# liuhuang31/Megatts2_HierSpeechpp

Hardware: AMD Instinct MI355X
Metric: 16kHz audio samples/sec (whole node) + RTF, HierSpeech++ vocoder batch=32 (higher is better)
Workload: dtype f32; 1 GPU; vocoder-only infer(): 32 utterances x 4 s per GPU (BASELINE.json configs[1]), synthetic weights; batch_per_gpu=32, frames=200, global_batch=32, parallelism=dp1 (contiguous utterance shards of the global batch, one RCCL weight broadcast), launch_mode=hipGraph replay of the captured step

## Files before the change

### megatts2_hierspeechpp_amd/csrc/hsp_dftseg.hip

```cpp
#include "hsp_device.h"
#include <algorithm>
#include <cmath>

namespace {
typedef float ds_f32x16 __attribute__((ext_vector_type(16)));
typedef float ds_f32x4 __attribute__((ext_vector_type(4)));
constexpr int DS_N = 128, DS_H = 64;
constexpr int DS_MEM = 256;
#define DS_ACC_ROW(r, half) (((r) & 3) + 8 * ((r) >> 2) + 4 * (half))

struct DsCol {
  int ch, p, s;
  bool ok;
};
__device__ __forceinline__ DsCol ds_col(int col, int ncols, int d, int S) {
  DsCol c;
  c.ok = col < ncols;
  const int cc = c.ok ? col : ncols - 1;
  const int per = d * S;
  c.ch = cc / per;
  const int rem = cc - c.ch * per;
  c.p = rem / S;
  c.s = rem - c.p * S;
  return c;
}

struct DsGeom {
  int cg, S, pitch, ngrp, nchunk, bufsz;
};
struct DsItem {
  int b, c0, ncg, s0, S;
};
__device__ __forceinline__ DsItem ds_item(int item, const hsp_dftseg_args& a, const DsGeom& G) {
  DsItem I;
  const int id = item / G.nchunk, sc = item - id * G.nchunk;
  I.b = id / G.ngrp;
  I.c0 = (id - I.b * G.ngrp) * G.cg;
  I.ncg = min(G.cg, a.C - I.c0);
  I.s0 = sc * G.S;
  I.S = min(G.S, a.nseg - I.s0);
  return I;
}
__device__ __forceinline__ void ds_barrier() { asm volatile("s_waitcnt lgkmcnt(0)\n\ts_barrier" ::: "memory"); }

__device__ __forceinline__ unsigned ds_lds_addr(const float* p) {
  return (unsigned)(size_t)(const __attribute__((address_space(3))) float*)p;
}
__device__ __forceinline__ void ds_rd(float& dst, unsigned addr) { asm volatile("ds_read_b32 %0, %1" : "=v"(dst) : "v"(addr)); }
template <int OFF>
__device__ __forceinline__ void ds_rd_at(float& dst, unsigned addr) {
  static_assert(OFF >= 0 && OFF < 65536, "ds_read immediate offsets are 16 bits");
// ... 53 lines not shown
  const float inv_ng = 1.0f / (float)s.ng;
#pragma unroll
  for (int u = 0; u < 16; ++u) {
    const int e = e0 + t + DS_MEM * u, ch = s.tot == s.ng ? 0 : ds_div(min(e, s.tot - 1), s.ng, inv_ng), gi = e - ch * s.ng;
    if (e < s.tot) *reinterpret_cast<ds_f32x4*>(buf + ch * G.pitch + s.sh - s.t0 + 4 * (s.g_lo + gi)) = v[u];
  }
}

constexpr int DA_SEG = 240, DA_RAW = 256, DA_A2 = 496, DA_SLICE = DA_RAW + DA_A2;
typedef float ds_f32x2 __attribute__((ext_vector_type(2)));
__device__ __forceinline__ void da_fence() { asm volatile("" ::: "memory"); }
struct DaItem {
  int pa, pb, pa4, nsg, nsegs;
};
template <bool RAG = false>
__device__ __forceinline__ DaItem da_item(const hsp_dftseg_args& a, const DsItem& I, const DsStage& s, int lb = 0) {
  const int L = RAG ? lb : a.L;
  DaItem A;
  A.pa = max(s.t0, 0);
  A.pb = min(s.t0 + s.len, L);
  A.pa4 = A.pa & ~3;
  A.nsg = (A.pb - A.pa4 + DA_SEG - 1) / DA_SEG;
  A.nsegs = I.ncg * A.nsg;
  if constexpr (RAG) {
    A.nsg = max(A.nsg, 1);
    A.nsegs = A.pb > A.pa ? I.ncg * A.nsg : 0;
  }
  return A;
}
template <bool RAG = false>
__device__ __forceinline__ ds_f32x4 da_load(const hsp_dftseg_args& a, const DsItem& I, const DaItem& A, int sI, int lane) {
  const int q = RAG ? max(min(sI, A.nsegs - 1), 0) : min(sI, A.nsegs - 1), ch = q / A.nsg, p0 = A.pa4 + DA_SEG * (q - ch * A.nsg);
  const float* xr = a.x + (int64_t)I.b * a.x_bs + (int64_t)(I.c0 + ch) * a.x_cs;
  return *reinterpret_cast<const ds_f32x4*>(xr + hsp_clampi(p0 - 8 + 4 * lane, 0, a.L - 4));
}
template <bool RAG = false>
__device__ __forceinline__ void da_segment(const hsp_dftseg_args& a, const DsGeom& G, const DsItem& I, const DsStage& s,
                                           const DaItem& A, int sI, int lane, ds_f32x4 rv, float* slice, float* buf,
                                           const float* flt, float add = 0.0f, int lb = 0, const float* last = nullptr,
                                           int64_t last_cs = 0) {
  const int ch = sI / A.nsg, p0 = A.pa4 + DA_SEG * (sI - ch * A.nsg);
  const int L = RAG ? lb : a.L;
  const int n_out = min(DA_SEG, L - p0);
  const int c = I.c0 + ch;
  const float kf = a.act_alpha_exp[c] * 0.318309886183790672f, kb = 0.5f * a.act_beta_inv[c];
  float* raw = slice;
  float* a2 = slice + DA_RAW;
  ds_f32x2 hu[6], hd[6];
#pragma unroll
  for (int i = 0; i < 6; ++i) {
    hu[i] = *reinterpret_cast<const ds_f32x2*>(flt + 2 * i);
    hd[i] = *reinterpret_cast<const ds_f32x2*>(flt + 12 + 2 * i);
  }
  {
    const int idx = p0 - 8 + 4 * lane;
    ds_f32x4 t = rv + add;
    t = idx < 0 ? ds_f32x4{t.x, t.x, t.x, t.x} : t;
    t = idx >= a.L ? ds_f32x4{t.w, t.w, t.w, t.w} : t;
    if constexpr (RAG) {
      const float rl = last[ch * last_cs] + add;
      t.x = idx >= L ? rl : t.x;
      t.y = idx + 1 >= L ? rl : t.y;
      t.z = idx + 2 >= L ? rl : t.z;
      t.w = idx + 3 >= L ? rl : t.w;
    }
    *reinterpret_cast<ds_f32x4*>(raw + 4 * lane) = t;
  }
  da_fence();
  const int npairs = (2 * n_out + 13) >> 2;
#pragma unroll
  for (int it = 0; it < 2; ++it) {
    const int pi = lane + 64 * it;
    if (pi < npairs) {
      const ds_f32x2* rp = reinterpret_cast<const ds_f32x2*>(raw + 2 * pi + 2);
      const ds_f32x2 r0 = rp[0], r1 = rp[1], r2 = rp[2], r3 = rp[3];
      const float xv[7] = {r0.y, r1.x, r1.y, r2.x, r2.y, r3.x, r3.y};
      ds_f32x2 u0 = {0.0f, 0.0f}, u1 = {0.0f, 0.0f};
#pragma unroll
      for (int i = 0; i < 6; ++i) {
        u0 = __builtin_elementwise_fma(ds_f32x2{xv[i], xv[i]}, hu[i], u0);
        u1 = __builtin_elementwise_fma(ds_f32x2{xv[i + 1], xv[i + 1]}, hu[i], u1);
      }
      *reinterpret_cast<ds_f32x4*>(a2 + 4 * pi) =
          ds_f32x4{hsp_snake_hw(u0.x, kf, kb), hsp_snake_hw(u0.y, kf, kb), hsp_snake_hw(u1.x, kf, kb), hsp_snake_hw(u1.y, kf, kb)};
    }
  }
  da_fence();
  if constexpr (RAG) {
    const int e = 2 * (L - p0) + 4;
    const bool tail = e < 2 * n_out + 9;
    if (p0 == 0 || tail) {
      if (p0 == 0 && lane < 5) a2[lane] = a2[5];
      if (tail && lane >= 8 && lane < 13) a2[e + lane - 7] = a2[e];
      da_fence();
    }
  } else if (p0 == 0 || p0 + n_out == a.L) {
    if (p0 == 0 && lane < 5) a2[lane] = a2[5];
    if (p0 + n_out == a.L && lane >= 8 && lane < 13) a2[2 * n_out + lane - 3] = a2[2 * n_out + 4];
    da_fence();
  }
  float* row = buf + ch * G.pitch + s.sh - s.t0;
#pragma unroll
  for (int it = 0; it < 2; ++it) {
    const int l2 = lane + 64 * it;
    if (2 * l2 < n_out) {
      const ds_f32x4* ap = reinterpret_cast<const ds_f32x4*>(a2 + 4 * l2);
      const ds_f32x4 q0 = ap[0], q1 = ap[1], q2 = ap[2];
      const ds_f32x2 q3 = *reinterpret_cast<const ds_f32x2*>(a2 + 4 * l2 + 12);
      const ds_f32x2 aw[7] = {{q0.x, q0.y}, {q0.z, q0.w}, {q1.x, q1.y}, {q1.z, q1.w}, {q2.x, q2.y}, {q2.z, q2.w}, q3};
      ds_f32x2 s0 = {0.0f, 0.0f}, s1 = {0.0f, 0.0f};
#pragma unroll
      for (int k = 0; k < 6; ++k) {
        s0 = __builtin_elementwise_fma(aw[k], hd[k], s0);
        s1 = __builtin_elementwise_fma(aw[k + 1], hd[k], s1);
      }
      const int p = p0 + 2 * l2;
      if (p >= A.pa && p < A.pb) row[p] = s0.x + s0.y;
      if (p + 1 >= A.pa && p + 1 < A.pb) row[p + 1] = s1.x + s1.y;
    }
  }
  da_fence();
}

template <bool ACT, bool RAG = false>
__global__ __launch_bounds__(DS_MEM) __attribute__((amdgpu_waves_per_eu(2, 2))) void dftseg_fwd_kernel(const hsp_dftseg_args a, const DsGeom G) {
  extern __shared__ __attribute__((aligned(16))) float lds[];
  const int tid = threadIdx.x, lane = tid & 63, wave = __builtin_amdgcn_readfirstlane(tid >> 6);
  const int l32 = lane & 31, half = lane >> 5;
  const int hop = DS_N - (a.k - 1), d = a.dil, pitch = G.pitch;
  const int nitems = a.B * G.ngrp * G.nchunk;
  const int nmine = (nitems - (int)blockIdx.x + (int)gridDim.x - 1) / (int)gridDim.x;
  const int wh = wave & 1, pairw = wave >> 1;
  float fa[32];
  {
    const float* frow = a.dft + (32 * wh + l32) * DS_H + half;
#pragma unroll
    for (int ks = 0; ks < 32; ++ks) fa[ks] = frow[2 * ks];
  }
  float* const twl = lds + G.bufsz;
  if (tid < 64) twl[tid] = a.dft[DS_H * DS_H + tid];
  float ov[32];
  bool pok = false;
  unsigned lb1 = 0, lb2 = 0, lbz = 0;
  const unsigned rowb = 4u * (unsigned)a.xf_bs, imb = 4u * (unsigned)(a.C * a.Np);
  const int lanek = 16 * wh + 4 * half;
  auto put = [&](int i) __attribute__((always_inline)) {
    const int r = i >> 2, w = i & 3;
    const unsigned cr = (unsigned)((r & 3) + 8 * (r >> 2)) * rowb;
    unsigned off = w < 2 ? lb1 + cr : lb2 - cr;
    if (r == 0 && w >= 2) off = lanek == 0 ? lbz : off;
    if (w & 1) off += imb;
    if (pok) *reinterpret_cast<float*>(reinterpret_cast<char*>(a.xf) + off) = ov[i];
  };
  const bool vec = ((a.L | (int)a.x_bs | (int)a.x_cs) & 3) == 0 && (reinterpret_cast<uintptr_t>(a.x) & 15) == 0;
  constexpr bool act = ACT;
  float* const flt = lds + G.bufsz + 64;
  float* const slice = flt + 32 + wave * DA_SLICE;
  if (act && tid < 24) {
    const int i = tid >> 1;
    flt[tid] = tid < 12 ? 2.0f * a.act_filt[10 - 2 * i + (tid & 1)] : a.act_filt[tid];
  }
  if (act) __syncthreads();
  DsItem I = ds_item(blockIdx.x, a, G);
  DsStage sg = ds_stage_of(a, I);
  auto row_len = [&](const DsItem& It) __attribute__((always_inline)) {
    return RAG ? (int)min(max(a.act_len[It.b], (int64_t)1), (int64_t)a.L) : a.L;
  };
  int lb = row_len(I);
  DaItem da = da_item<RAG>(a, I, sg, lb);
  ds_f32x4 pv[16];
  auto prefetch = [&]() __attribute__((always_inline)) {
    if (act) {
#pragma unroll
      for (int i = 0; i < 16; ++i) pv[i] = da_load<RAG>(a, I, da, wave + 4 * i, lane);
    } else if (vec) {
      ds_stage_load(a, I, sg, 0, tid, pv);
    }
  };
  prefetch();
  for (int it = 0; it < nmine; ++it) {
    if (it) ds_barrier();
    if (act) {
      const float* last = RAG ? a.x + (int64_t)I.b * a.x_bs + (int64_t)I.c0 * a.x_cs + (lb - 1) : nullptr;
#pragma unroll
      for (int i = 0; i < 16; ++i)
        if (wave + 4 * i < da.nsegs)
          da_segment<RAG>(a, G, I, sg, da, wave + 4 * i, lane, pv[i], slice, lds, flt, 0.0f, lb, last, a.x_cs);
      for (int sI = wave + 64; sI < da.nsegs; sI += 4)
        da_segment<RAG>(a, G, I, sg, da, sI, lane, da_load<RAG>(a, I, da, sI, lane), slice, lds, flt, 0.0f, lb, last, a.x_cs);
      for (int ch = 0; ch < I.ncg; ++ch) {
        float* row = lds + ch * pitch + sg.sh;
        for (int j = tid; j < min(-sg.t0, sg.len); j += DS_MEM) row[j] = 0.0f;
        for (int j = max((RAG ? lb : a.L) - sg.t0, 0) + tid; j < sg.len; j += DS_MEM) row[j] = 0.0f;
      }
    } else if (vec) {
      ds_stage_write(G, sg, 0, tid, lds, pv);
      for (int e0 = DS_MEM * 16; e0 < sg.tot; e0 += DS_MEM * 16) {
        ds_f32x4 v[16];
        ds_stage_load(a, I, sg, e0, tid, v);
        ds_stage_write(G, sg, e0, tid, lds, v);
      }
      for (int ch = 0; ch < I.ncg; ++ch) {
        float* row = lds + ch * pitch + sg.sh;
        for (int j = tid; j < min(-sg.t0, sg.len); j += DS_MEM) row[j] = 0.0f;
        for (int j = max(a.L - sg.t0, 0) + tid; j < sg.len; j += DS_MEM) row[j] = 0.0f;
      }
    } else {
      for (int ch = 0; ch < I.ncg; ++ch) {
        const float* xr = a.x + (int64_t)I.b * a.x_bs + (int64_t)(I.c0 + ch) * a.x_cs;
        float* row = lds + ch * pitch + sg.sh;
        for (int j0 = 0; j0 < sg.len; j0 += DS_MEM * 16) {
          float v[16];
#pragma unroll
          for (int u = 0; u < 16; ++u) v[u] = xr[min(max(sg.t0 + j0 + tid + DS_MEM * u, 0), a.L - 1)];
#pragma unroll
          for (int u = 0; u < 16; ++u) {
            const int j = j0 + tid + DS_MEM * u, ti = sg.t0 + j;
            if (j < sg.len) row[j] = (ti >= 0 && ti < a.L) ? v[u] : 0.0f;
          }
        }
      }
    }
    ds_barrier();
    const DsItem Ic = I;
    const int shc = sg.sh;
    if (it + 1 < nmine) {
      I = ds_item(blockIdx.x + (it + 1) * gridDim.x, a, G);
      sg = ds_stage_of(a, I);
      lb = row_len(I);
      da = da_item<RAG>(a, I, sg, lb);
      prefetch();
    }
    const int S = Ic.S, ncols = Ic.ncg * d * S;
    const float ipc = 1.0f / (float)(d * S), isc = 1.0f / (float)S;
    const float* buf = lds + shc;
    const int step = 4 * d;
    for (int cb = 32 * pairw; cb < ncols; cb += 64) {
      const DsCol q = ds_col_f(cb + l32, ncols, d, S, ipc, isc);
      const float* bp = buf + q.ch * pitch + q.p + d * (q.s * hop + 2 * half);
      ds_f32x16 ae, ao;
#pragma unroll
      for (int r = 0; r < 16; ++r) ae[r] = ao[r] = 0.0f;
      float rb[2][8];
      unsigned pe = ds_lds_addr(bp), po = pe + 4u * d;
      const unsigned st = 4u * step;
      auto issue = [&](float (&r)[8]) __attribute__((always_inline)) {
#pragma unroll
        for (int j = 0; j < 4; ++j) {
          ds_rd(r[2 * j], pe);
          ds_rd(r[2 * j + 1], po);
          pe += st;
          po += st;
        }
      };
      issue(rb[0]);
#pragma unroll
      for (int g = 0; g < 8; ++g) {
        ds_wait<0>(rb[g & 1]);
        if (g + 1 < 8) issue(rb[(g + 1) & 1]);
#pragma unroll
        for (int j = 0; j < 4; ++j) {
          ae = __builtin_amdgcn_mfma_f32_32x32x2f32(fa[4 * g + j], rb[g & 1][2 * j], ae, 0, 0, 0);
          ao = __builtin_amdgcn_mfma_f32_32x32x2f32(fa[4 * g + j], rb[g & 1][2 * j + 1], ao, 0, 0, 0);
          put(4 * g + j);
        }
      }
#pragma unroll
      for (int r = 0; r < 8; ++r) {
        const float er = ae[r], ei = ae[r + 8], orr = ao[r], oi = ao[r + 8];
        const float wc = twl[lanek + (r & 3) + 8 * (r >> 2)], ws = twl[32 + lanek + (r & 3) + 8 * (r >> 2)];
        const float tr = wc * orr + ws * oi, ti = wc * oi - ws * orr;
        const bool z = r == 0 && wh == 0 && half == 0;
        const bool z3 = z && a.prod3;
        ov[4 * r + 0] = z3 ? -er : er + tr;
        ov[4 * r + 1] = z ? (a.prod3 ? -tr : er - tr) : ei + ti;
        ov[4 * r + 2] = z ? ei : er - tr;
        ov[4 * r + 3] = z ? -oi : ti - ei;
      }
      {
        const unsigned colb = 4u * (unsigned)((Ic.c0 + q.ch) * a.Np + (Ic.b * d + q.p) * a.nseg + Ic.s0 + q.s);
        pok = q.ok;
        lb1 = colb + (unsigned)lanek * rowb;
        lb2 = colb + (unsigned)(64 - lanek) * rowb;
        lbz = colb + 32u * rowb;
      }
    }
  }
#pragma unroll
  for (int i = 0; i < 32; ++i) put(i);
}


template <int W, int U, bool RES, bool ACC>
__device__ __forceinline__ void ds_inv_epilogue_t(const hsp_dftseg_args& a, const DsGeom& G, const DsItem& I, const float* buf,
                                                  int w, int nw, int lane, int tb, int tl) {
  typedef float vec_t __attribute__((ext_vector_type(W)));
  const int nel = tl / W;
  const int R = (nel + 64 * U - 1) / (64 * U);
  const float ps = a.post_scale;
  int ch = 0, rr = w;
  while (rr >= R) rr -= R, ++ch;
  while (ch < I.ncg) {
    const int c = I.c0 + ch;
    const float bz = a.bias ? a.bias[c] : 0.0f;
// ... 176 lines not shown
    else ds_inv_epilogue<1, 4>(a, G, I, lds, wave, 4, lane, tb, tl);
    if (++it_c < nmine) {
      blk_c = 0;
      I = item_of(it_c);
      ncols = I.ncg * d * I.S;
    } else {
      done = true;
    }
  };
  float v1[16], v2[16];
  DsCol q1, q2;
  fetch_next(v1, q1);
  fetch_next(v2, q2);
  while (true) {
    step(v1, q1);
    if (done) break;
    step(v2, q2);
    if (done) break;
  }
}

struct DpGeom {
  int cg, ngrp, S1, pitchA, S2, pitchB, offB, offX, offT;
};

template <bool RAG = false>
__global__ __launch_bounds__(512) __attribute__((amdgpu_waves_per_eu(2, 2))) void dftseg_pair_kernel(
    const hsp_dftseg_args ai, const hsp_dftseg_args af, const DpGeom G) {
  extern __shared__ __attribute__((aligned(16))) float lds[];
  const int tid = threadIdx.x, lane = tid & 63, wave = __builtin_amdgcn_readfirstlane(tid >> 6);
  const int l32 = lane & 31, half = lane >> 5;
  const int hop1 = DS_N - (ai.k - 1), d1 = ai.dil, hop2 = DS_N - (af.k - 1), d2 = af.dil;
  float* const sA = lds;
  float* const sB = lds + G.offB;
  float* const twl = lds + G.offT;
  float* const flt = twl + 64;
  const int grp = wave >> 2, w4 = wave & 3, wh1 = w4 & 1, eo = w4 >> 1;
  const int pw = wave >> 1, wh3 = wave & 1;
  float* const bbuf = lds + G.offX + grp * (128 * 32);
  float* const slice = lds + G.offX + wave * DA_SLICE;
  float fa1[32], fa3[32], twc[4], tws[4];
  {
    const float* frow = ai.dft + (32 * wh1 + l32) * DS_H + half;
#pragma unroll
    for (int ks = 0; ks < 32; ++ks) fa1[ks] = frow[2 * ks];
    const float* grow = af.dft + (32 * wh3 + l32) * DS_H + half;
#pragma unroll
    for (int ks = 0; ks < 32; ++ks) fa3[ks] = grow[2 * ks];
// ... 64 lines not shown
#pragma unroll
      for (int ks = 0; ks < 32; ks += 2) {
        acc = __builtin_amdgcn_mfma_f32_32x32x2f32(fa1[ks], bp[ks * 64], acc, 0, 0, 0);
        acc2 = __builtin_amdgcn_mfma_f32_32x32x2f32(fa1[ks + 1], bp[ks * 64 + 64], acc2, 0, 0, 0);
      }
      if (q.ok) ds_inv_scatter(sA + q.ch * G.pitchA + q.p + d1 * (q.s * hop1 + i0), d1, i0, hop1, wh1, acc, acc2);
      ds_barrier();
    };
    for (int st = 0; st < nst; ++st) {
      if (odd) step1(v2, q2);
      else step1(v1, q1);
      odd = !odd;
    }
    {
      DsStage sg;
      sg.t0 = -af.pad;
      sg.len = d2 * ((G.S2 - 1) * hop2 + DS_N);
      sg.sh = 4 + (sg.t0 & 3);
      sg.g_lo = 0;
      sg.ng = 0;
      sg.tot = 0;
      const int lb = RAG ? (int)min(max(af.act_len[I.b], (int64_t)1), (int64_t)af.L) : af.L;
      const DaItem da = da_item<RAG>(af, I, sg, lb);
      for (int sI = wave; sI < da.nsegs; sI += 8) {
        const int ch = sI / da.nsg, p0 = da.pa4 + DA_SEG * (sI - ch * da.nsg);
        const ds_f32x4 rv = *reinterpret_cast<const ds_f32x4*>(sA + ch * G.pitchA + hsp_clampi(p0 - 8 + 4 * lane, 0, af.L - 4));
        da_segment<RAG>(af, Gf, I, sg, da, sI, lane, rv, slice, sB, flt, ai.bias ? ai.bias[I.c0 + ch] : 0.0f,
                        lb, sA + (lb - 1), G.pitchA);
      }
      for (int ch = 0; ch < I.ncg; ++ch) {
        float* row = sB + ch * G.pitchB + sg.sh;
        for (int j = tid; j < min(-sg.t0, sg.len); j += 512) row[j] = 0.0f;
        for (int j = max(lb - sg.t0, 0) + tid; j < sg.len; j += 512) row[j] = 0.0f;
      }
      ds_barrier();
      const int ncols2 = I.ncg * d2 * G.S2;
      const float* buf = sB + sg.sh;
      const int step = 4 * d2;
      const unsigned rowb = 4u * (unsigned)af.xf_bs, imb = 4u * (unsigned)(af.C * af.Np);
      const int lanek = 16 * wh3 + 4 * half;
      const float ip2 = 1.0f / (float)(d2 * G.S2), is2 = 1.0f / (float)G.S2;
      for (int cb = 32 * pw; cb < ncols2; cb += 128) {
        const DsCol q = ds_col_f(cb + l32, ncols2, d2, G.S2, ip2, is2);
        const float* bp = buf + q.ch * G.pitchB + q.p + d2 * (q.s * hop2 + 2 * half);
        ds_f32x16 ae, ao;
#pragma unroll
        for (int r = 0; r < 16; ++r) ae[r] = ao[r] = 0.0f;
#pragma unroll
        for (int ks = 0; ks < 32; ++ks) {
          ae = __builtin_amdgcn_mfma_f32_32x32x2f32(fa3[ks], bp[ks * step], ae, 0, 0, 0);
          ao = __builtin_amdgcn_mfma_f32_32x32x2f32(fa3[ks], bp[ks * step + d2], ao, 0, 0, 0);
        }
        if (q.ok) {
          const unsigned colb = 4u * (unsigned)((I.c0 + q.ch) * af.Np + (I.b * d2 + q.p) * af.nseg + q.s);
          char* const base = reinterpret_cast<char*>(af.xf);
#pragma unroll
          for (int r = 0; r < 8; ++r) {
            const int kr = (r & 3) + 8 * (r >> 2);
            const float er = ae[r], ei = ae[r + 8], orr = ao[r], oi = ao[r + 8];
            const float wc = twl[lanek + kr], ws = twl[32 + lanek + kr];
            const float tr = wc * orr + ws * oi, ti = wc * oi - ws * orr;
            const bool z = r == 0 && lanek == 0;
            const bool z3 = z && af.prod3;
            const unsigned o1 = colb + (unsigned)(lanek + kr) * rowb;
            const unsigned o2 = colb + (z ? 32u : (unsigned)(64 - lanek - kr)) * rowb;
            *reinterpret_cast<float*>(base + o1) = z3 ? -er : er + tr;
            *reinterpret_cast<float*>(base + o1 + imb) = z ? (af.prod3 ? -tr : er - tr) : ei + ti;
            *reinterpret_cast<float*>(base + o2) = z ? ei : er - tr;
            *reinterpret_cast<float*>(base + o2 + imb) = z ? -oi : ti - ei;
          }
        }
      }
    }
  }
}

int ds_check(const hsp_dftseg_args& a) {
  if (!a.xf || !a.dft || a.B <= 0 || a.C <= 0 || a.L <= 0 || a.k < 2 || a.k > 64 || a.dil < 1 || a.dil > 8) return HSP_EINVAL;
  const int hop = DS_N - (a.k - 1);
  const int per_phase = (a.L + a.dil - 1) / a.dil;
  if (a.nseg != (per_phase + hop - 1) / hop || a.pad < 0 || a.pad > (a.k - 1) * a.dil) return HSP_EINVAL;
  if ((int64_t)a.B * a.dil * a.nseg > a.Np || a.xf_bs < (int64_t)2 * a.C * a.Np) return HSP_EINVAL;
  if (a.xf_bs * 64 * 4 > 0xffffffffll) return HSP_EINVAL;
  return 0;
}

int64_t ds_resident(size_t lds_bytes) {
  static int cus = 0;
  if (!cus) {
    int dev = 0, n = 0;
    if (hipGetDevice(&dev) != hipSuccess || hipDeviceGetAttribute(&n, hipDeviceAttributeMultiprocessorCount, dev) != hipSuccess || n <= 0)
      n = 256;
    cus = n;
  }
  const int per = (int)std::min<size_t>(2, std::max<size_t>(1, (160 * 1024) / std::max<size_t>(lds_bytes, 1)));
  return (int64_t)cus * per;
}

DsGeom ds_geom(const hsp_dftseg_args& a, bool inverse) {
  const int hop = DS_N - (a.k - 1), d = a.dil;
  const int budget = inverse ? 16384 : 17408;
  auto row_of = [&](int S) { return inverse ? ((d * S * hop + 3) & ~3) : ((d * ((S - 1) * hop + DS_N) + 12 + 3) & ~3); };
  int S = a.nseg;
  if (row_of(S) > budget) {
    int smax = inverse ? budget / (d * hop) : ((budget - 15) / d - DS_N) / hop + 1;
    smax &= ~1;
    if (smax < 2) smax = 2;
    const int nch = (a.nseg + smax - 1) / smax;
    S = ((a.nseg + nch - 1) / nch + 1) & ~1;
    if (S > smax) S = smax;
  }
  DsGeom G;
  G.S = S;
  G.pitch = row_of(S);
  int cmax = budget / G.pitch;
  cmax = cmax < 1 ? 1 : (cmax > 32 ? 32 : cmax);
  cmax = cmax > a.C ? a.C : cmax;
  const int quantum = inverse ? 32 : 64;
  const int nchunk = (a.nseg + S - 1) / S;
  int best = cmax;
  double best_score = 0.0;
  for (int cg = cmax; cg >= (cmax + 1) / 2; --cg) {
    const int ncols = cg * d * S;
    const double fill = (double)ncols / (quantum * ((ncols + quantum - 1) / quantum));
    const size_t lds = inverse ? ((size_t)cg * G.pitch + 128 * 32) * sizeof(float) : ((size_t)cg * G.pitch + 64 + 32 + 4 * DA_SLICE) * sizeof(float);
    const int64_t res = ds_resident(lds), items = (int64_t)a.B * ((a.C + cg - 1) / cg) * nchunk;
    const double balance = (double)items / (double)(((items + res - 1) / res) * res);
    const double score = fill * balance;
    if (score > best_score + 1e-9) best_score = score, best = cg;
  }
  G.cg = best;
  G.bufsz = (G.cg * G.pitch + 3) & ~3;
  G.nchunk = (a.nseg + S - 1) / S;
  G.ngrp = (a.C + G.cg - 1) / G.cg;
  return G;
// ... 24 lines not shown
      const int64_t items = (int64_t)ai.B * ((ai.C + c - 1) / c);
      const double score = fill * (double)items / (double)(((items + res - 1) / res) * res);
      if (score > best_score + 1e-9) best_score = score, best = c;
    }
    cg = best;
  }
  G.cg = cg;
  G.ngrp = (ai.C + cg - 1) / cg;
  G.offB = cg * G.pitchA;
  G.offX = G.offB + cg * G.pitchB;
  G.offT = G.offX + 2 * 128 * 32;
  return G;
}
int ds_limits(const hsp_dftseg_args& a, bool act) {
  const DsGeom Gf = ds_geom(a, false), Gi = ds_geom(a, true);
  const size_t lds_f = ((size_t)Gf.bufsz + 64 + (act ? 32 + 4 * DA_SLICE : 0)) * sizeof(float);
  const size_t lds_i = ((size_t)Gi.bufsz + 128 * 32) * sizeof(float);
  if (lds_f > 160 * 1024 || lds_i > 160 * 1024) return HSP_EINVAL;
  if ((int64_t)a.B * Gf.ngrp * Gf.nchunk > 0x7fffffff || (int64_t)a.B * Gi.ngrp * Gi.nchunk > 0x7fffffff) return HSP_EINVAL;
  return 0;
}
}

extern "C" int hsp_dftseg_supported(const hsp_dftseg_args* ap) {
  if (!ap) return 0;
  hsp_dftseg_args a = *ap;
  static const float dummy = 0.0f;
  a.xf = const_cast<float*>(&dummy);
  a.dft = &dummy;
  return ds_check(a) == 0 && ds_limits(a, true) == 0 ? 1 : 0;
}

extern "C" int hsp_dftseg_tables_f32(float* fwd, float* inv) {
  if (!fwd || !inv) return HSP_EINVAL;
  const double w = 2.0 * 3.14159265358979323846 / DS_H;
  for (int wh = 0; wh < 2; ++wh)
    for (int j = 0; j < 32; ++j) {
      const int k = 16 * wh + (j & 15);
      float* row = fwd + (32 * wh + j) * DS_H;
      for (int n = 0; n < DS_H; ++n)
        row[n] = (float)(j < 16 ? cos(w * k * n) : (k == 0 ? ((n & 1) ? -1.0 : 1.0) : -sin(w * k * n)));
    }
  for (int j = 0; j < DS_H; ++j)
    for (int t = 0; t < DS_H; ++t) {
      const int k = t & 31;
      double v;
      if (k == 0) v = (t == 0 ? 1.0 : ((j & 1) ? -1.0 : 1.0)) / 128.0;
      else v = (t < 32 ? cos(w * k * j) : -sin(w * k * j)) / 64.0;
      inv[j * DS_H + t] = (float)v;
    }
  for (int k = 0; k < 32; ++k) {
    fwd[DS_H * DS_H + k] = inv[DS_H * DS_H + k] = (float)cos(w * k / 2);
    fwd[DS_H * DS_H + 32 + k] = inv[DS_H * DS_H + 32 + k] = (float)sin(w * k / 2);
  }
  return 0;
}

extern "C" int hsp_dftseg_fwd_f32(const hsp_dftseg_args* ap, void* stream) {
  if (!ap || !ap->x) return HSP_EINVAL;
  const hsp_dftseg_args& a = *ap;
  if (int e = ds_check(a)) return e;
  const DsGeom G = ds_geom(a, false);
  const bool act = a.act_alpha_exp != nullptr;
  if (act && (!a.act_beta_inv || !a.act_filt || ((a.L | (int)a.x_bs | (int)a.x_cs) & 3) || (reinterpret_cast<uintptr_t>(a.x) & 15)))
    return HSP_EINVAL;
  const size_t lds_bytes = ((size_t)G.bufsz + 64 + (act ? 32 + 4 * DA_SLICE : 0)) * sizeof(float);
  const int64_t items = (int64_t)a.B * G.ngrp * G.nchunk;
  if (lds_bytes > 160 * 1024 || items > 0x7fffffff) return HSP_EINVAL;
  const int64_t blocks = std::min<int64_t>(items, ds_resident(lds_bytes));
  if (a.act_len && !act) return HSP_EINVAL;
  if (a.act_len) {
    static hsp_lds_flags flags_rag;
    if (lds_bytes > 32 * 1024)
      if (int e = hsp_raise_lds_limit(reinterpret_cast<const void*>(dftseg_fwd_kernel<true, true>), 160 * 1024, flags_rag))
        return e;
    hipLaunchKernelGGL((dftseg_fwd_kernel<true, true>), dim3((unsigned)blocks), dim3(DS_MEM), lds_bytes,
                       static_cast<hipStream_t>(stream), a, G);
    return (int)hipGetLastError();
  }
  static hsp_lds_flags flags[2];
  const void* kern = act ? reinterpret_cast<const void*>(dftseg_fwd_kernel<true>) : reinterpret_cast<const void*>(dftseg_fwd_kernel<false>);
  if (lds_bytes > 32 * 1024)
    if (int e = hsp_raise_lds_limit(kern, 160 * 1024, flags[act])) return e;
  if (act)
    hipLaunchKernelGGL(dftseg_fwd_kernel<true>, dim3((unsigned)blocks), dim3(DS_MEM), lds_bytes, static_cast<hipStream_t>(stream), a, G);
  else
    hipLaunchKernelGGL(dftseg_fwd_kernel<false>, dim3((unsigned)blocks), dim3(DS_MEM), lds_bytes, static_cast<hipStream_t>(stream), a, G);
  return (int)hipGetLastError();
}

extern "C" int hsp_dftseg_inv_f32(const hsp_dftseg_args* ap, void* stream) {
  if (!ap || !ap->y) return HSP_EINVAL;
  const hsp_dftseg_args& a = *ap;
  if (int e = ds_check(a)) return e;
  const DsGeom G = ds_geom(a, true);
  const int nbuf = ((size_t)G.bufsz + 2 * 128 * 32) * sizeof(float) <= 80 * 1024 ? 2 : 1;
  const size_t lds_bytes = ((size_t)G.bufsz + nbuf * 128 * 32) * sizeof(float);
  const int64_t items = (int64_t)a.B * G.ngrp * G.nchunk;
  if (lds_bytes > 160 * 1024 || items > 0x7fffffff) return HSP_EINVAL;
  const int64_t blocks = std::min<int64_t>(items, ds_resident(lds_bytes));
  static hsp_lds_flags flags;
  if (lds_bytes > 32 * 1024)
    if (int e = hsp_raise_lds_limit(reinterpret_cast<const void*>(dftseg_inv_kernel), 160 * 1024, flags)) return e;
  hipLaunchKernelGGL(dftseg_inv_kernel, dim3((unsigned)blocks), dim3(DS_MEM), lds_bytes, static_cast<hipStream_t>(stream), a, G,
                     nbuf);
  return (int)hipGetLastError();
}

extern "C" int hsp_dftseg_pair_supported(const hsp_dftseg_args* inv, const hsp_dftseg_args* fwd) {
  return inv && fwd && dp_geom(*inv, *fwd).cg > 0 ? 1 : 0;
}

extern "C" int hsp_dftseg_pair_f32(const hsp_dftseg_args* inv, const hsp_dftseg_args* fwd, void* stream) {
  if (!inv || !fwd) return HSP_EINVAL;
  const DpGeom G = dp_geom(*inv, *fwd);
  if (G.cg < 1) return HSP_EINVAL;
  const size_t lds_bytes = (size_t)(G.offT + 96) * sizeof(float);
  const int64_t items = (int64_t)inv->B * G.ngrp;
  if (lds_bytes > 160 * 1024 || items > 0x7fffffff) return HSP_EINVAL;
  const int64_t blocks = std::min<int64_t>(items, ds_resident(lds_bytes));
  if (fwd->act_len) {
    static hsp_lds_flags flags_rag;
    if (int e = hsp_raise_lds_limit(reinterpret_cast<const void*>(dftseg_pair_kernel<true>), 160 * 1024, flags_rag)) return e;
    hipLaunchKernelGGL(dftseg_pair_kernel<true>, dim3((unsigned)blocks), dim3(512), lds_bytes, static_cast<hipStream_t>(stream),
                       *inv, *fwd, G);
    return (int)hipGetLastError();
  }
  static hsp_lds_flags flags;
  if (int e = hsp_raise_lds_limit(reinterpret_cast<const void*>(dftseg_pair_kernel<false>), 160 * 1024, flags)) return e;
  hipLaunchKernelGGL(dftseg_pair_kernel<false>, dim3((unsigned)blocks), dim3(512), lds_bytes, static_cast<hipStream_t>(stream), *inv,
                     *fwd, G);
  return (int)hipGetLastError();
}
```

Before: 35.47 million samples/s.

## Specialize DFT-segment kernels on dilation and interior segments, hoist per-channel params

Templates the forward and pair DFT-segment kernels on dilation (1, 3, 5), so the MFMA LDS reads use compile-time offsets. Adds an interior-segment fast path that skips edge clamping and tail fixups and writes vectorized pairs. Replaces per-segment divisions with an incremental channel/slice counter and loads snake alpha/beta and bias only when the channel changes. Also adds debug knobs gated behind HSP_TUNING, which grows code size and template instantiations.

```diff
diff --git a/megatts2_hierspeechpp_amd/csrc/hsp_dftseg.hip b/megatts2_hierspeechpp_amd/csrc/hsp_dftseg.hip
--- a/megatts2_hierspeechpp_amd/csrc/hsp_dftseg.hip
+++ b/megatts2_hierspeechpp_amd/csrc/hsp_dftseg.hip
@@ -1,6 +1,7 @@
 #include "hsp_device.h"
 #include <algorithm>
 #include <cmath>
+#include <cstdlib>
 
 namespace {
 typedef float ds_f32x16 __attribute__((ext_vector_type(16)));
@@ -8,6 +9,14 @@
 constexpr int DS_N = 128, DS_H = 64;
 constexpr int DS_MEM = 256;
 #define DS_ACC_ROW(r, half) (((r) & 3) + 8 * ((r) >> 2) + 4 * (half))
+enum { DS_DBG_ACT_COPY = 1, DS_DBG_NO_MFMA = 2, DS_DBG_NO_STORE = 4, DS_DBG_NO_TAIL = 8 };
+#ifdef HSP_TUNING
+#define DS_DBG(dbg, bit) (((dbg) & (bit)) != 0)
+#define DS_GEOM_DBG(G) ((G).dbg)
+#else
+#define DS_DBG(dbg, bit) false
+#define DS_GEOM_DBG(G) 0
+#endif
 
 struct DsCol {
   int ch, p, s;
@@ -27,6 +36,9 @@
 
 struct DsGeom {
   int cg, S, pitch, ngrp, nchunk, bufsz;
+#ifdef HSP_TUNING
+  int dbg;
+#endif
 };
 struct DsItem {
   int b, c0, ncg, s0, S;
@@ -126,28 +138,43 @@
   A.pa4 = A.pa & ~3;
   A.nsg = (A.pb - A.pa4 + DA_SEG - 1) / DA_SEG;
   A.nsegs = I.ncg * A.nsg;
-  if constexpr (RAG) {
-    A.nsg = max(A.nsg, 1);
-    A.nsegs = A.pb > A.pa ? I.ncg * A.nsg : 0;
-  }
+  A.nsg = max(A.nsg, 1);
+  if constexpr (RAG) A.nsegs = A.pb > A.pa ? I.ncg * A.nsg : 0;
   return A;
 }
-template <bool RAG = false>
-__device__ __forceinline__ ds_f32x4 da_load(const hsp_dftseg_args& a, const DsItem& I, const DaItem& A, int sI, int lane) {
-  const int q = RAG ? max(min(sI, A.nsegs - 1), 0) : min(sI, A.nsegs - 1), ch = q / A.nsg, p0 = A.pa4 + DA_SEG * (q - ch * A.nsg);
+struct DaPos {
+  int ch, sl;
+};
+__device__ __forceinline__ DaPos da_pos(int sI, int nsg) {
+  DaPos p = {0, sI};
+  while (p.sl >= nsg) p.sl -= nsg, ++p.ch;
+  return p;
+}
+__device__ __forceinline__ void da_advance(DaPos& p, int n, int nsg) {
+  p.sl += n;
+  while (p.sl >= nsg) p.sl -= nsg, ++p.ch;
+}
+__device__ __forceinline__ ds_f32x4 da_load(const hsp_dftseg_args& a, const DsItem& I, const DaItem& A, DaPos P, int lane) {
+  const bool in = P.ch * A.nsg + P.sl < A.nsegs;
+  const int ch = in ? P.ch : (A.nsegs > 0 ? I.ncg - 1 : 0), sl = in ? P.sl : (A.nsegs > 0 ? A.nsg - 1 : 0);
+  const int p0 = A.pa4 + DA_SEG * sl;
   const float* xr = a.x + (int64_t)I.b * a.x_bs + (int64_t)(I.c0 + ch) * a.x_cs;
   return *reinterpret_cast<const ds_f32x4*>(xr + hsp_clampi(p0 - 8 + 4 * lane, 0, a.L - 4));
 }
-template <bool RAG = false>
-__device__ __forceinline__ void da_segment(const hsp_dftseg_args& a, const DsGeom& G, const DsItem& I, const DsStage& s,
-                                           const DaItem& A, int sI, int lane, ds_f32x4 rv, float* slice, float* buf,
-                                           const float* flt, float add = 0.0f, int lb = 0, const float* last = nullptr,
-                                           int64_t last_cs = 0) {
-  const int ch = sI / A.nsg, p0 = A.pa4 + DA_SEG * (sI - ch * A.nsg);
+struct DaChan {
+  float kf, kb;
+};
+__device__ __forceinline__ DaChan da_chan(const hsp_dftseg_args& a, int c) {
+  return {a.act_alpha_exp[c] * 0.318309886183790672f, 0.5f * a.act_beta_inv[c]};
+}
+template <bool RAG, bool INT>
+__device__ __forceinline__ void da_segment_t(const hsp_dftseg_args& a, const DsGeom& G, const DsStage& s, const DaItem& A,
+                                             int ch, int p0, DaChan K, int lane, ds_f32x4 rv, float* slice, float* buf,
+                                             const float* flt, float add, int lb, const float* last, int64_t last_cs, int dbg) {
   const int L = RAG ? lb : a.L;
-  const int n_out = min(DA_SEG, L - p0);
-  const int c = I.c0 + ch;
-  const float kf = a.act_alpha_exp[c] * 0.318309886183790672f, kb = 0.5f * a.act_beta_inv[c];
+  const int n_out = INT ? DA_SEG : min(DA_SEG, L - p0);
+  constexpr bool interior = INT;
+  const float kf = K.kf, kb = K.kb;
   float* raw = slice;
   float* a2 = slice + DA_RAW;
   ds_f32x2 hu[6], hd[6];
@@ -157,16 +184,18 @@
     hd[i] = *reinterpret_cast<const ds_f32x2*>(flt + 12 + 2 * i);
   }
   {
-    const int idx = p0 - 8 + 4 * lane;
     ds_f32x4 t = rv + add;
-    t = idx < 0 ? ds_f32x4{t.x, t.x, t.x, t.x} : t;
-    t = idx >= a.L ? ds_f32x4{t.w, t.w, t.w, t.w} : t;
-    if constexpr (RAG) {
-      const float rl = last[ch * last_cs] + add;
-      t.x = idx >= L ? rl : t.x;
-      t.y = idx + 1 >= L ? rl : t.y;
-      t.z = idx + 2 >= L ? rl : t.z;
-      t.w = idx + 3 >= L ? rl : t.w;
+    if constexpr (!interior) {
+      const int idx = p0 - 8 + 4 * lane;
+      t = idx < 0 ? ds_f32x4{t.x, t.x, t.x, t.x} : t;
+      t = idx >= a.L ? ds_f32x4{t.w, t.w, t.w, t.w} : t;
+      if constexpr (RAG) {
+        const float rl = last[ch * last_cs] + add;
+        t.x = idx >= L ? rl : t.x;
+        t.y = idx + 1 >= L ? rl : t.y;
+        t.z = idx + 2 >= L ? rl : t.z;
+        t.w = idx + 3 >= L ? rl : t.w;
+      }
     }
     *reinterpret_cast<ds_f32x4*>(raw + 4 * lane) = t;
   }
@@ -179,18 +208,23 @@
       const ds_f32x2* rp = reinterpret_cast<const ds_f32x2*>(raw + 2 * pi + 2);
       const ds_f32x2 r0 = rp[0], r1 = rp[1], r2 = rp[2], r3 = rp[3];
       const float xv[7] = {r0.y, r1.x, r1.y, r2.x, r2.y, r3.x, r3.y};
-      ds_f32x2 u0 = {0.0f, 0.0f}, u1 = {0.0f, 0.0f};
-#pragma unroll
-      for (int i = 0; i < 6; ++i) {
-        u0 = __builtin_elementwise_fma(ds_f32x2{xv[i], xv[i]}, hu[i], u0);
-        u1 = __builtin_elementwise_fma(ds_f32x2{xv[i + 1], xv[i + 1]}, hu[i], u1);
-      }
-      *reinterpret_cast<ds_f32x4*>(a2 + 4 * pi) =
-          ds_f32x4{hsp_snake_hw(u0.x, kf, kb), hsp_snake_hw(u0.y, kf, kb), hsp_snake_hw(u1.x, kf, kb), hsp_snake_hw(u1.y, kf, kb)};
+      if (DS_DBG(dbg, DS_DBG_ACT_COPY)) {
+        *reinterpret_cast<ds_f32x4*>(a2 + 4 * pi) = ds_f32x4{xv[2], xv[3], xv[4], xv[5]};
+      } else {
+        ds_f32x2 u0 = {0.0f, 0.0f}, u1 = {0.0f, 0.0f};
+#pragma unroll
+        for (int i = 0; i < 6; ++i) {
+          u0 = __builtin_elementwise_fma(ds_f32x2{xv[i], xv[i]}, hu[i], u0);
+          u1 = __builtin_elementwise_fma(ds_f32x2{xv[i + 1], xv[i + 1]}, hu[i], u1);
+        }
+        *reinterpret_cast<ds_f32x4*>(a2 + 4 * pi) =
+            ds_f32x4{hsp_snake_hw(u0.x, kf, kb), hsp_snake_hw(u0.y, kf, kb), hsp_snake_hw(u1.x, kf, kb), hsp_snake_hw(u1.y, kf, kb)};
+      }
     }
   }
   da_fence();
-  if constexpr (RAG) {
+  if constexpr (INT) {
+  } else if constexpr (RAG) {
     const int e = 2 * (L - p0) + 4;
     const bool tail = e < 2 * n_out + 9;
     if (p0 == 0 || tail) {
@@ -212,26 +246,91 @@
       const ds_f32x4 q0 = ap[0], q1 = ap[1], q2 = ap[2];
       const ds_f32x2 q3 = *reinterpret_cast<const ds_f32x2*>(a2 + 4 * l2 + 12);
       const ds_f32x2 aw[7] = {{q0.x, q0.y}, {q0.z, q0.w}, {q1.x, q1.y}, {q1.z, q1.w}, {q2.x, q2.y}, {q2.z, q2.w}, q3};
-      ds_f32x2 s0 = {0.0f, 0.0f}, s1 = {0.0f, 0.0f};
-#pragma unroll
-      for (int k = 0; k < 6; ++k) {
-        s0 = __builtin_elementwise_fma(aw[k], hd[k], s0);
-        s1 = __builtin_elementwise_fma(aw[k + 1], hd[k], s1);
+      ds_f32x2 o = aw[3];
+      if (!DS_DBG(dbg, DS_DBG_ACT_COPY)) {
+        ds_f32x2 s0 = {0.0f, 0.0f}, s1 = {0.0f, 0.0f};
+#pragma unroll
+        for (int k = 0; k < 6; ++k) {
+          s0 = __builtin_elementwise_fma(aw[k], hd[k], s0);
+          s1 = __builtin_elementwise_fma(aw[k + 1], hd[k], s1);
+        }
+        o = ds_f32x2{s0.x + s0.y, s1.x + s1.y};
       }
       const int p = p0 + 2 * l2;
-      if (p >= A.pa && p < A.pb) row[p] = s0.x + s0.y;
-      if (p + 1 >= A.pa && p + 1 < A.pb) row[p + 1] = s1.x + s1.y;
+      if constexpr (interior) {
+        *reinterpret_cast<ds_f32x2*>(row + p) = o;
+      } else {
+        if (p >= A.pa && p < A.pb) row[p] = o.x;
+        if (p + 1 >= A.pa && p + 1 < A.pb) row[p + 1] = o.y;
+      }
     }
   }
   da_fence();
 }
-
-template <bool ACT, bool RAG = false>
+template <bool RAG = false>
+__device__ __forceinline__ void da_segment(const hsp_dftseg_args& a, const DsGeom& G, const DsStage& s, const DaItem& A,
+                                           int ch, int p0, DaChan K, int lane, ds_f32x4 rv, float* slice, float* buf,
+                                           const float* flt, float add = 0.0f, int lb = 0, const float* last = nullptr,
+                                           int64_t last_cs = 0, int dbg = 0) {
+  const int L = RAG ? lb : a.L;
+  if (p0 >= 8 && p0 + DA_SEG + 8 <= L && p0 >= A.pa && p0 + DA_SEG <= A.pb)
+    da_segment_t<RAG, true>(a, G, s, A, ch, p0, K, lane, rv, slice, buf, flt, add, lb, last, last_cs, dbg);
+  else
+    da_segment_t<RAG, false>(a, G, s, A, ch, p0, K, lane, rv, slice, buf, flt, add, lb, last, last_cs, dbg);
+}
+
+template <int D, int G>
+__device__ __forceinline__ void ds_fwd_issue(float (&r)[8], unsigned& pe, unsigned& po, unsigned st) {
+  if constexpr (D != 0) {
+    ds_rd_at<16 * D * (4 * G + 0)>(r[0], pe);
+    ds_rd_at<16 * D * (4 * G + 0) + 4 * D>(r[1], pe);
+    ds_rd_at<16 * D * (4 * G + 1)>(r[2], pe);
+    ds_rd_at<16 * D * (4 * G + 1) + 4 * D>(r[3], pe);
+    ds_rd_at<16 * D * (4 * G + 2)>(r[4], pe);
+    ds_rd_at<16 * D * (4 * G + 2) + 4 * D>(r[5], pe);
+    ds_rd_at<16 * D * (4 * G + 3)>(r[6], pe);
+    ds_rd_at<16 * D * (4 * G + 3) + 4 * D>(r[7], pe);
+  } else {
+#pragma unroll
+    for (int j = 0; j < 4; ++j) {
+      ds_rd(r[2 * j], pe);
+      ds_rd(r[2 * j + 1], po);
+      pe += st;
+      po += st;
+    }
+  }
+}
+template <int D, int G, typename Put>
+__device__ __forceinline__ void ds_fwd_groups(const float (&fa)[32], float (&rb)[2][8], unsigned& pe, unsigned& po, unsigned st,
+                                              ds_f32x16& ae, ds_f32x16& ao, bool mfma, Put& put) {
+  ds_wait<0>(rb[G & 1]);
+  if constexpr (G + 1 < 8) ds_fwd_issue<D, G + 1>(rb[(G + 1) & 1], pe, po, st);
+#pragma unroll
+  for (int j = 0; j < 4; ++j) {
+    if (mfma) {
+      ae = __builtin_amdgcn_mfma_f32_32x32x2f32(fa[4 * G + j], rb[G & 1][2 * j], ae, 0, 0, 0);
+      ao = __builtin_amdgcn_mfma_f32_32x32x2f32(fa[4 * G + j], rb[G & 1][2 * j + 1], ao, 0, 0, 0);
+    }
+    put(4 * G + j);
+  }
+  if constexpr (G + 1 < 8) ds_fwd_groups<D, G + 1>(fa, rb, pe, po, st, ae, ao, mfma, put);
+}
+template <int D, typename Put>
+__device__ __forceinline__ void ds_fwd_block(const float (&fa)[32], const float* bp, int d, ds_f32x16& ae, ds_f32x16& ao, bool mfma,
+                                             Put& put) {
+  float rb[2][8];
+  unsigned pe = ds_lds_addr(bp), po = pe + 4u * d;
+  const unsigned st = 16u * d;
+  ds_fwd_issue<D, 0>(rb[0], pe, po, st);
+  ds_fwd_groups<D, 0>(fa, rb, pe, po, st, ae, ao, mfma, put);
+}
+
+template <bool ACT, bool RAG = false, int D = 0>
 __global__ __launch_bounds__(DS_MEM) __attribute__((amdgpu_waves_per_eu(2, 2))) void dftseg_fwd_kernel(const hsp_dftseg_args a, const DsGeom G) {
   extern __shared__ __attribute__((aligned(16))) float lds[];
   const int tid = threadIdx.x, lane = tid & 63, wave = __builtin_amdgcn_readfirstlane(tid >> 6);
   const int l32 = lane & 31, half = lane >> 5;
-  const int hop = DS_N - (a.k - 1), d = a.dil, pitch = G.pitch;
+  const int hop = DS_N - (a.k - 1), d = D ? D : a.dil, pitch = G.pitch;
   const int nitems = a.B * G.ngrp * G.nchunk;
   const int nmine = (nitems - (int)blockIdx.x + (int)gridDim.x - 1) / (int)gridDim.x;
   const int wh = wave & 1, pairw = wave >> 1;
@@ -275,8 +374,12 @@
   ds_f32x4 pv[16];
   auto prefetch = [&]() __attribute__((always_inline)) {
     if (act) {
-#pragma unroll
-      for (int i = 0; i < 16; ++i) pv[i] = da_load<RAG>(a, I, da, wave + 4 * i, lane);
+      DaPos P = da_pos(wave, da.nsg);
+#pragma unroll
+      for (int i = 0; i < 16; ++i) {
+        pv[i] = da_load(a, I, da, P, lane);
+        da_advance(P, 4, da.nsg);
+      }
     } else if (vec) {
       ds_stage_load(a, I, sg, 0, tid, pv);
     }
@@ -286,12 +389,22 @@
     if (it) ds_barrier();
     if (act) {
       const float* last = RAG ? a.x + (int64_t)I.b * a.x_bs + (int64_t)I.c0 * a.x_cs + (lb - 1) : nullptr;
-#pragma unroll
-      for (int i = 0; i < 16; ++i)
-        if (wave + 4 * i < da.nsegs)
-          da_segment<RAG>(a, G, I, sg, da, wave + 4 * i, lane, pv[i], slice, lds, flt, 0.0f, lb, last, a.x_cs);
-      for (int sI = wave + 64; sI < da.nsegs; sI += 4)
-        da_segment<RAG>(a, G, I, sg, da, sI, lane, da_load<RAG>(a, I, da, sI, lane), slice, lds, flt, 0.0f, lb, last, a.x_cs);
+      DaPos P = da_pos(wave, da.nsg);
+      int chk = -1;
+      DaChan K = {0.0f, 0.0f};
+      auto seg = [&](ds_f32x4 rv) __attribute__((always_inline)) {
+        if (P.ch != chk) K = da_chan(a, I.c0 + P.ch), chk = P.ch;
+        da_segment<RAG>(a, G, sg, da, P.ch, da.pa4 + DA_SEG * P.sl, K, lane, rv, slice, lds, flt, 0.0f, lb, last, a.x_cs, DS_GEOM_DBG(G));
+      };
+#pragma unroll
+      for (int i = 0; i < 16; ++i) {
+        if (wave + 4 * i < da.nsegs) seg(pv[i]);
+        da_advance(P, 4, da.nsg);
+      }
+      for (int sI = wave + 64; sI < da.nsegs; sI += 4) {
+        seg(da_load(a, I, da, P, lane));
+        da_advance(P, 4, da.nsg);
+      }
       for (int ch = 0; ch < I.ncg; ++ch) {
         float* row = lds + ch * pitch + sg.sh;
         for (int j = tid; j < min(-sg.t0, sg.len); j += DS_MEM) row[j] = 0.0f;
@@ -338,37 +451,15 @@
     const int S = Ic.S, ncols = Ic.ncg * d * S;
     const float ipc = 1.0f / (float)(d * S), isc = 1.0f / (float)S;
     const float* buf = lds + shc;
-    const int step = 4 * d;
-    for (int cb = 32 * pairw; cb < ncols; cb += 64) {
+    const bool mfma = !DS_DBG(DS_GEOM_DBG(G), DS_DBG_NO_MFMA);
+    const int ncb = DS_DBG(DS_GEOM_DBG(G), DS_DBG_NO_TAIL) && ncols >= 32 ? ncols & ~31 : ncols;
+    for (int cb = 32 * pairw; cb < ncb; cb += 64) {
       const DsCol q = ds_col_f(cb + l32, ncols, d, S, ipc, isc);
       const float* bp = buf + q.ch * pitch + q.p + d * (q.s * hop + 2 * half);
       ds_f32x16 ae, ao;
 #pragma unroll
       for (int r = 0; r < 16; ++r) ae[r] = ao[r] = 0.0f;
-      float rb[2][8];
-      unsigned pe = ds_lds_addr(bp), po = pe + 4u * d;
-      const unsigned st = 4u * step;
-      auto issue = [&](float (&r)[8]) __attribute__((always_inline)) {
-#pragma unroll
-        for (int j = 0; j < 4; ++j) {
-          ds_rd(r[2 * j], pe);
-          ds_rd(r[2 * j + 1], po);
-          pe += st;
-          po += st;
-        }
-      };
-      issue(rb[0]);
-#pragma unroll
-      for (int g = 0; g < 8; ++g) {
-        ds_wait<0>(rb[g & 1]);
-        if (g + 1 < 8) issue(rb[(g + 1) & 1]);
-#pragma unroll
-        for (int j = 0; j < 4; ++j) {
-          ae = __builtin_amdgcn_mfma_f32_32x32x2f32(fa[4 * g + j], rb[g & 1][2 * j], ae, 0, 0, 0);
-          ao = __builtin_amdgcn_mfma_f32_32x32x2f32(fa[4 * g + j], rb[g & 1][2 * j + 1], ao, 0, 0, 0);
-          put(4 * g + j);
-        }
-      }
+      ds_fwd_block<D>(fa, bp, d, ae, ao, mfma, put);
 #pragma unroll
       for (int r = 0; r < 8; ++r) {
         const float er = ae[r], ei = ae[r + 8], orr = ao[r], oi = ao[r + 8];
@@ -383,7 +474,7 @@
       }
       {
         const unsigned colb = 4u * (unsigned)((Ic.c0 + q.ch) * a.Np + (Ic.b * d + q.p) * a.nseg + Ic.s0 + q.s);
-        pok = q.ok;
+        pok = q.ok && !DS_DBG(DS_GEOM_DBG(G), DS_DBG_NO_STORE);
         lb1 = colb + (unsigned)lanek * rowb;
         lb2 = colb + (unsigned)(64 - lanek) * rowb;
         lbz = colb + 32u * rowb;
@@ -606,8 +697,20 @@
 
 struct DpGeom {
   int cg, ngrp, S1, pitchA, S2, pitchB, offB, offX, offT;
+#ifdef HSP_TUNING
+  int dbg;
+#endif
 };
 
+template <int D>
+__device__ __forceinline__ void dp_fwd_mfma(const float (&fa)[32], const float* bp, int d, ds_f32x16& ae, ds_f32x16& ao) {
+  const int dd = D ? D : d;
+#pragma unroll
+  for (int ks = 0; ks < 32; ++ks) {
+    ae = __builtin_amdgcn_mfma_f32_32x32x2f32(fa[ks], bp[ks * 4 * dd], ae, 0, 0, 0);
+    ao = __builtin_amdgcn_mfma_f32_32x32x2f32(fa[ks], bp[ks * 4 * dd + dd], ao, 0, 0, 0);
+  }
+}
 template <bool RAG = false>
 __global__ __launch_bounds__(512) __attribute__((amdgpu_waves_per_eu(2, 2))) void dftseg_pair_kernel(
     const hsp_dftseg_args ai, const hsp_dftseg_args af, const DpGeom G) {
@@ -718,11 +821,20 @@
       sg.tot = 0;
       const int lb = RAG ? (int)min(max(af.act_len[I.b], (int64_t)1), (int64_t)af.L) : af.L;
       const DaItem da = da_item<RAG>(af, I, sg, lb);
+      DaPos P = da_pos(wave, da.nsg);
+      int chk = -1;
+      DaChan K = {0.0f, 0.0f};
+      float bias1 = 0.0f;
       for (int sI = wave; sI < da.nsegs; sI += 8) {
-        const int ch = sI / da.nsg, p0 = da.pa4 + DA_SEG * (sI - ch * da.nsg);
+        const int ch = P.ch, p0 = da.pa4 + DA_SEG * P.sl;
         const ds_f32x4 rv = *reinterpret_cast<const ds_f32x4*>(sA + ch * G.pitchA + hsp_clampi(p0 - 8 + 4 * lane, 0, af.L - 4));
-        da_segment<RAG>(af, Gf, I, sg, da, sI, lane, rv, slice, sB, flt, ai.bias ? ai.bias[I.c0 + ch] : 0.0f,
-                        lb, sA + (lb - 1), G.pitchA);
+        if (ch != chk) {
+          K = da_chan(af, I.c0 + ch);
+          bias1 = ai.bias ? ai.bias[I.c0 + ch] : 0.0f;
+          chk = ch;
+        }
+        da_segment<RAG>(af, Gf, sg, da, ch, p0, K, lane, rv, slice, sB, flt, bias1, lb, sA + (lb - 1), G.pitchA, DS_GEOM_DBG(G));
+        da_advance(P, 8, da.nsg);
       }
       for (int ch = 0; ch < I.ncg; ++ch) {
         float* row = sB + ch * G.pitchB + sg.sh;
@@ -732,22 +844,23 @@
       ds_barrier();
       const int ncols2 = I.ncg * d2 * G.S2;
       const float* buf = sB + sg.sh;
-      const int step = 4 * d2;
+      const bool mfma = !DS_DBG(DS_GEOM_DBG(G), DS_DBG_NO_MFMA);
+      const int ncb2 = DS_DBG(DS_GEOM_DBG(G), DS_DBG_NO_TAIL) && ncols2 >= 32 ? ncols2 & ~31 : ncols2;
       const unsigned rowb = 4u * (unsigned)af.xf_bs, imb = 4u * (unsigned)(af.C * af.Np);
       const int lanek = 16 * wh3 + 4 * half;
       const float ip2 = 1.0f / (float)(d2 * G.S2), is2 = 1.0f / (float)G.S2;
-      for (int cb = 32 * pw; cb < ncols2; cb += 128) {
+      for (int cb = 32 * pw; cb < ncb2; cb += 128) {
         const DsCol q = ds_col_f(cb + l32, ncols2, d2, G.S2, ip2, is2);
         const float* bp = buf + q.ch * G.pitchB + q.p + d2 * (q.s * hop2 + 2 * half);
         ds_f32x16 ae, ao;
 #pragma unroll
         for (int r = 0; r < 16; ++r) ae[r] = ao[r] = 0.0f;
-#pragma unroll
-        for (int ks = 0; ks < 32; ++ks) {
-          ae = __builtin_amdgcn_mfma_f32_32x32x2f32(fa3[ks], bp[ks * step], ae, 0, 0, 0);
-          ao = __builtin_amdgcn_mfma_f32_32x32x2f32(fa3[ks], bp[ks * step + d2], ao, 0, 0, 0);
-        }
-        if (q.ok) {
+        if (!mfma) {
+        } else if (d2 == 1) dp_fwd_mfma<1>(fa3, bp, d2, ae, ao);
+        else if (d2 == 3) dp_fwd_mfma<3>(fa3, bp, d2, ae, ao);
+        else if (d2 == 5) dp_fwd_mfma<5>(fa3, bp, d2, ae, ao);
+        else dp_fwd_mfma<0>(fa3, bp, d2, ae, ao);
+        if (q.ok && !DS_DBG(DS_GEOM_DBG(G), DS_DBG_NO_STORE)) {
           const unsigned colb = 4u * (unsigned)((I.c0 + q.ch) * af.Np + (I.b * d2 + q.p) * af.nseg + q.s);
           char* const base = reinterpret_cast<char*>(af.xf);
 #pragma unroll
@@ -771,6 +884,13 @@
   }
 }
 
+#ifdef HSP_TUNING
+int ds_tune_dbg() {
+  const char* e = getenv("HSP_TUNE_DFTSEG");
+  return e ? atoi(e) : 0;
+}
+#endif
+
 int ds_check(const hsp_dftseg_args& a) {
   if (!a.xf || !a.dft || a.B <= 0 || a.C <= 0 || a.L <= 0 || a.k < 2 || a.k > 64 || a.dil < 1 || a.dil > 8) return HSP_EINVAL;
   const int hop = DS_N - (a.k - 1);
@@ -806,7 +926,7 @@
     S = ((a.nseg + nch - 1) / nch + 1) & ~1;
     if (S > smax) S = smax;
   }
-  DsGeom G;
+  DsGeom G = {};
   G.S = S;
   G.pitch = row_of(S);
   int cmax = budget / G.pitch;
@@ -877,6 +997,26 @@
 }
 }
 
+namespace {
+template <bool ACT, bool RAG, int D>
+int ds_fwd_launch(const hsp_dftseg_args& a, const DsGeom& G, unsigned blocks, size_t lds_bytes, void* stream) {
+  static hsp_lds_flags flags;
+  if (lds_bytes > 32 * 1024)
+    if (int e = hsp_raise_lds_limit(reinterpret_cast<const void*>(dftseg_fwd_kernel<ACT, RAG, D>), 160 * 1024, flags)) return e;
+  hipLaunchKernelGGL((dftseg_fwd_kernel<ACT, RAG, D>), dim3(blocks), dim3(DS_MEM), lds_bytes, static_cast<hipStream_t>(stream), a, G);
+  return (int)hipGetLastError();
+}
+template <bool ACT, bool RAG>
+int ds_fwd_launch_d(const hsp_dftseg_args& a, const DsGeom& G, unsigned blocks, size_t lds_bytes, void* stream) {
+  switch (a.dil) {
+    case 1: return ds_fwd_launch<ACT, RAG, 1>(a, G, blocks, lds_bytes, stream);
+    case 3: return ds_fwd_launch<ACT, RAG, 3>(a, G, blocks, lds_bytes, stream);
+    case 5: return ds_fwd_launch<ACT, RAG, 5>(a, G, blocks, lds_bytes, stream);
+    default: return ds_fwd_launch<ACT, RAG, 0>(a, G, blocks, lds_bytes, stream);
+  }
+}
+}
+
 extern "C" int hsp_dftseg_supported(const hsp_dftseg_args* ap) {
   if (!ap) return 0;
   hsp_dftseg_args a = *ap;
@@ -915,7 +1055,10 @@
   if (!ap || !ap->x) return HSP_EINVAL;
   const hsp_dftseg_args& a = *ap;
   if (int e = ds_check(a)) return e;
-  const DsGeom G = ds_geom(a, false);
+  DsGeom G = ds_geom(a, false);
+#ifdef HSP_TUNING
+  G.dbg = ds_tune_dbg();
+#endif
   const bool act = a.act_alpha_exp != nullptr;
   if (act && (!a.act_beta_inv || !a.act_filt || ((a.L | (int)a.x_bs | (int)a.x_cs) & 3) || (reinterpret_cast<uintptr_t>(a.x) & 15)))
     return HSP_EINVAL;
@@ -924,31 +1067,19 @@
   if (lds_bytes > 160 * 1024 || items > 0x7fffffff) return HSP_EINVAL;
   const int64_t blocks = std::min<int64_t>(items, ds_resident(lds_bytes));
   if (a.act_len && !act) return HSP_EINVAL;
-  if (a.act_len) {
-    static hsp_lds_flags flags_rag;
-    if (lds_bytes > 32 * 1024)
-      if (int e = hsp_raise_lds_limit(reinterpret_cast<const void*>(dftseg_fwd_kernel<true, true>), 160 * 1024, flags_rag))
-        return e;
-    hipLaunchKernelGGL((dftseg_fwd_kernel<true, true>), dim3((unsigned)blocks), dim3(DS_MEM), lds_bytes,
-                       static_cast<hipStream_t>(stream), a, G);
-    return (int)hipGetLastError();
-  }
-  static hsp_lds_flags flags[2];
-  const void* kern = act ? reinterpret_cast<const void*>(dftseg_fwd_kernel<true>) : reinterpret_cast<const void*>(dftseg_fwd_kernel<false>);
-  if (lds_bytes > 32 * 1024)
-    if (int e = hsp_raise_lds_limit(kern, 160 * 1024, flags[act])) return e;
-  if (act)
-    hipLaunchKernelGGL(dftseg_fwd_kernel<true>, dim3((unsigned)blocks), dim3(DS_MEM), lds_bytes, static_cast<hipStream_t>(stream), a, G);
-  else
-    hipLaunchKernelGGL(dftseg_fwd_kernel<false>, dim3((unsigned)blocks), dim3(DS_MEM), lds_bytes, static_cast<hipStream_t>(stream), a, G);
-  return (int)hipGetLastError();
+  const unsigned nb = (unsigned)blocks;
+  if (a.act_len) return ds_fwd_launch_d<true, true>(a, G, nb, lds_bytes, stream);
+  return act ? ds_fwd_launch_d<true, false>(a, G, nb, lds_bytes, stream) : ds_fwd_launch_d<false, false>(a, G, nb, lds_bytes, stream);
 }
 
 extern "C" int hsp_dftseg_inv_f32(const hsp_dftseg_args* ap, void* stream) {
   if (!ap || !ap->y) return HSP_EINVAL;
   const hsp_dftseg_args& a = *ap;
   if (int e = ds_check(a)) return e;
-  const DsGeom G = ds_geom(a, true);
+  DsGeom G = ds_geom(a, true);
+#ifdef HSP_TUNING
+  G.dbg = 0;
+#endif
   const int nbuf = ((size_t)G.bufsz + 2 * 128 * 32) * sizeof(float) <= 80 * 1024 ? 2 : 1;
   const size_t lds_bytes = ((size_t)G.bufsz + nbuf * 128 * 32) * sizeof(float);
   const int64_t items = (int64_t)a.B * G.ngrp * G.nchunk;
@@ -968,8 +1099,11 @@
 
 extern "C" int hsp_dftseg_pair_f32(const hsp_dftseg_args* inv, const hsp_dftseg_args* fwd, void* stream) {
   if (!inv || !fwd) return HSP_EINVAL;
-  const DpGeom G = dp_geom(*inv, *fwd);
+  DpGeom G = dp_geom(*inv, *fwd);
   if (G.cg < 1) return HSP_EINVAL;
+#ifdef HSP_TUNING
+  G.dbg = ds_tune_dbg();
+#endif
   const size_t lds_bytes = (size_t)(G.offT + 96) * sizeof(float);
   const int64_t items = (int64_t)inv->B * G.ngrp;
   if (lds_bytes > 160 * 1024 || items > 0x7fffffff) return HSP_EINVAL;
```

After: 35.95 million samples/s, median of 6. 1.01x the previous value.
